# wei-zeng98/piano-a2s

Measured on AMD Instinct MI355X. Metric: training clips/sec (12 s, 5-bar), higher is better.
Workload: dtype f32

## Files before the change

piano_a2s_amd/csrc/a2s_api.hip:

```cpp
#define A2S_SWITCHES_IMPL
#include "a2s_internal.h"

thread_local char a2s_err_msg[512] = {0};
long long a2s_launch_counter = 0;

#define ST ((hipStream_t)stream)

extern "C" {

const char* a2s_last_error(void) { return a2s_err_msg; }
int a2s_version(void) { return 1; }
long long a2s_launch_count(void) { return __atomic_load_n(&a2s_launch_counter, __ATOMIC_RELAXED); }

int a2s_gemm_f32(void* stream, int M, int N, int K, float alpha, const float* A, long sAm, long sAk, const float* B, long sBk,
                 long sBn, float beta, float* C, long ldc, const float* bias, int act, int batch, long bsA, long bsB, long bsC,
                 int splitk, float* workspace, size_t workspace_bytes) {
    return a2s_gemm_impl(ST, M, N, K, alpha, A, sAm, sAk, B, sBk, sBn, beta, C, ldc, bias, act, batch, bsA, bsB, bsC, splitk,
                         workspace, workspace_bytes);
}
int a2s_gemm_f32_affine(void* stream, int M, int N, int K, float alpha, const float* A, long sAm, long sAk, const float* B, long sBk,
                        long sBn, float beta, float* C, long ldc, const float* bias, int act, int batch, long bsA, long bsB, long bsC,
                        int splitk, float* workspace, size_t workspace_bytes, const float* a_scale, const float* a_shift, int a_period,
                        const float* b_scale, const float* b_shift, int b_period) {
    return a2s_gemm_affine_impl(ST, M, N, K, alpha, A, sAm, sAk, B, sBk, sBn, beta, C, ldc, bias, act, batch, bsA, bsB, bsC, splitk,
// ... 42 lines not shown
}
int a2s_linear_fwd_eligible(int M, int N, int K, int period) { return a2s_linear_fwd_ok(M, N, K, 4, 4, period, nullptr, nullptr, nullptr) ? 1 : 0; }
int a2s_linear_dgrad_blocks(int M) { return a2s_linear_dgrad_blocks_impl(M); }
int a2s_linear_dgrad_eligible(int M, int N, int K, int period) {
    return a2s_linear_dgrad_ok(M, N, K, 4, 1, K, 4, period, nullptr, nullptr, nullptr, nullptr) ? 1 : 0;
}
int a2s_gemm_f32_bnstats(void* stream, int M, int N, int K, const float* A, long sAm, long sAk, const float* B, long sBk, long sBn, float* C, long ldc,
                         const float* y, const float* mean, const float* invstd, const float* scale, const float* shift, int period, float* partial) {
    return a2s_gemm_affine_impl(ST, M, N, K, 1.f, A, sAm, sAk, B, sBk, sBn, 0.f, C, ldc, nullptr, 0, 1, 0, 0, 0, 1, nullptr, 0,
                                nullptr, nullptr, 0, nullptr, nullptr, 0, y, mean, invstd, scale, shift, partial, period, 0, nullptr, nullptr);
}
int a2s_gemm_bnstats_blocks(int M, int period) { return a2s_cdiv(M, 128) * a2s_gemm_bnstats_slots(period); }
size_t a2s_gemm_workspace_bytes(int M, int N, int batch, int splitk) { return a2s_gemm_workspace_bytes_impl(M, N, batch, splitk); }
int a2s_gemm_pick_splitk(int M, int N, int K, int batch) { return a2s_gemm_pick_splitk_impl(M, N, K, batch); }
void a2s_gemm_debug_tile(int cfg) { a2s_gemm_debug_tile_impl(cfg); }
size_t a2s_note_step_workspace_floats(int H, int E) { return a2s_note_step_workspace_floats_impl(H, E); }
int a2s_debug_set(const char* key, int value) {
    if (!key) return A2S_ERR_ARG;
    const int id = a2s_switch_find(key);
    if (id >= 0) { a2s_switch_store(id, value); return A2S_OK; }
    if (!strcmp(key, "attn_deferred_fast")) { a2s_attn_deferred_fast = value ? 1 : 0; return A2S_OK; }
    if (!strcmp(key, "tallk_wgrad")) { a2s_tallk_wgrad_on = value ? 1 : 0; return A2S_OK; }
    if (!strcmp(key, "tallk_wgrad_max_splits")) { a2s_tallk_wgrad_max_splits = value > 0 ? value : 0; return A2S_OK; }
    if (!strcmp(key, "gemm_tile")) { a2s_gemm_debug_tile_impl(value); return A2S_OK; }
    snprintf(a2s_err_msg, sizeof(a2s_err_msg), "a2s_debug_set: unknown key %s", key);
    return A2S_ERR_ARG;
}
int a2s_env_check(void) {
    if (const char* e = a2s_switch_env_error()) A2S_FAIL(A2S_ERR_ARG, "%s: expected a decimal number >= 0", e);
    return A2S_OK;
}

int a2s_persist_abort_latch(void* device_word) { a2s_persist_latch_set(device_word); return A2S_OK; }

int a2s_debug_get(const char* key) {
    if (!key) return -1;
    const int id = a2s_switch_find(key);
    if (id == A2S_SW_attn_pair_fused_rows) return a2s_attn_pair_fused_rows();
    if (id >= 0) return a2s_sw((a2s_switch)id);
    if (!strcmp(key, "attn_pair_launches")) return (int)a2s_attn_pair_launches();
    if (!strcmp(key, "attn_pair_bwd_launches")) return (int)a2s_attn_pair_bwd_launches();
    if (!strcmp(key, "attn_deferred_fast")) return a2s_attn_deferred_fast;
    if (!strcmp(key, "tallk_wgrad")) return a2s_tallk_wgrad_on;
    if (!strcmp(key, "tallk_wgrad_max_splits")) return a2s_tallk_wgrad_max_splits;
    if (!strcmp(key, "tallk_wgrad_launches")) return (int)a2s_tallk_wgrad_launches();
    if (!strcmp(key, "attn_dk_ahead_launches")) return (int)a2s_attn_dk_ahead_launches();
    if (!strcmp(key, "attn_denc_launches")) return (int)a2s_attn_denc_launches();
    if (!strcmp(key, "dec_mid_launches")) return a2s_dec_mid_launches();
    if (!strcmp(key, "dec_cmb_launches")) return a2s_dec_cmb_launches();
    if (!strcmp(key, "dec_persist_launches")) return a2s_dec_persist_launches();
    if (!strcmp(key, "edit_distance_launches")) return (int)a2s_edit_distance_launches();
    if (!strcmp(key, "conv_rows16_c20_launches")) return (int)a2s_conv_rows16_c20_launches();
    if (!strcmp(key, "device_cus")) return a2s_device_geometry().cus;
    if (!strcmp(key, "device_xccs")) return a2s_device_geometry().xccs;
    return -1;
}

int a2s_conv3x3(void* stream, const float* x, const float* w, float* y, const float* in_scale, const float* in_shift,
                float* stat_partial, int B, int T, int F, int Cin, int Cout, int flip, float* workspace) {
    return a2s_conv3x3_impl(ST, x, w, y, in_scale, in_shift, stat_partial, B, T, F, Cin, Cout, flip, workspace, nullptr, nullptr, nullptr, nullptr, nullptr, nullptr,
                            nullptr, nullptr);
}
int a2s_conv3x3_ranged(void* stream, const float* x, const float* w, float* y, const float* in_scale, const float* in_shift, const float* in_absmax,
                       float* stat_partial, float* out_absmax, int B, int T, int F, int Cin, int Cout, float* workspace) {
    return a2s_conv3x3_impl(ST, x, w, y, in_scale, in_shift, stat_partial, B, T, F, Cin, Cout, 0, workspace, nullptr, nullptr, nullptr, nullptr, nullptr, nullptr,
                            in_absmax, out_absmax);
}
int a2s_conv3x3_dgrad_bnstats(void* stream, const float* dy, const float* w, float* g, const float* yl, const float* yl_mean, const float* yl_invstd,
                              const float* yl_scale, const float* yl_shift, float* stat_partial, int B, int T, int F, int Cin, int Cout,
                              float* workspace) {
    if (!yl) { snprintf(a2s_err_msg, sizeof(a2s_err_msg), "conv3x3_dgrad_bnstats: yl is required"); return A2S_ERR_ARG; }
    return a2s_conv3x3_impl(ST, dy, w, g, nullptr, nullptr, stat_partial, B, T, F, Cin, Cout, 1, workspace, yl, yl_mean, yl_invstd, yl_scale, yl_shift, nullptr, nullptr, nullptr);
// ... 382 lines not shown
```

piano_a2s_amd/csrc/a2s_bwd.hip:

```cpp
#include "a2s_internal.h"

__global__ __launch_bounds__(256) void log_softmax_bwd_rows(const float* __restrict__ g, const float* __restrict__ y,
                                                            long outer_stride, int inner, float* __restrict__ dx,
                                                            int R, int V, int n_outer, int time_major) {
    const int row = blockIdx.x * 4 + (threadIdx.x >> 6), lane = threadIdx.x & 63;
    if (row >= R) return;
    const int ob = row / inner, in = row % inner;
    const float* gr = g + (long)ob * outer_stride + (long)in * V;
    const float* yr = y + (long)ob * outer_stride + (long)in * V;
    float s = 0.f;
    for (int j = lane; j < V; j += 64) s += gr[j];
    s = wave_sum(s);
    const long orow = time_major ? ((long)in * n_outer + ob) : row;
    for (int j = lane; j < V; j += 64) dx[orow * V + j] = gr[j] - expf(yr[j]) * s;
}

int a2s_log_softmax_bwd_rows_impl(hipStream_t st, const float* g, const float* y, long outer_stride, int inner, float* dx,
                                  int R, int V, int n_outer, int time_major) {
    hipLaunchKernelGGL(log_softmax_bwd_rows, dim3(a2s_cdiv(R, 4)), dim3(256), 0, st, g, y, outer_stride, inner, dx, R, V, n_outer, time_major);
    A2S_CHECK_LAUNCH("log_softmax_bwd_rows");
    return A2S_OK;
}

__global__ void gru_gates_bwd(const float* __restrict__ dh_a, long lda, const float* __restrict__ dh_b, long ldb,
// ... 378 lines not shown
    hipLaunchKernelGGL(embed_scatter_add, dim3(a2s_cdiv((long)R * E, 256)), dim3(256), 0, st, table_grad, ids64, ids32, id_stride,
                       const_id, g, ldg, col0, R, E, drop, inv_keep);
    A2S_CHECK_LAUNCH("embed_scatter_add");
    return A2S_OK;
}

__global__ void ew_act_bwd(const float* __restrict__ g, const float* __restrict__ y, float* __restrict__ dx, long n, int act) {
    const long stride = (long)gridDim.x * blockDim.x;
    for (long i = (long)blockIdx.x * blockDim.x + threadIdx.x; i < n; i += stride) {
        const float yy = y[i];
        dx[i] = act == 2 ? g[i] * (1.f - yy * yy) : (yy > 0.f ? g[i] : 0.f);
    }
}
int a2s_ew_act_bwd_impl(hipStream_t st, const float* g, const float* y, float* dx, long n, int act) {
    hipLaunchKernelGGL(ew_act_bwd, dim3(min((long)2048, (n + 255) / 256)), dim3(256), 0, st, g, y, dx, n, act);
    A2S_CHECK_LAUNCH("ew_act_bwd");
    return A2S_OK;
}


static int attn_pair_bwd_sweep(hipStream_t st, const a2s_note_dec_bwd_args& au, const a2s_note_dec_bwd_args& al, int s, AttnPairStep& p);
static int attn_pair_bwd_combine(hipStream_t st, const a2s_note_dec_bwd_args& a, int s, const AttnPairStep& p);

struct NoteBwdStaff { bool mid = false; int cur = 0; int fused_rows_limit = -1; };
static int note_bwd_step_rows(const a2s_note_dec_bwd_args& a, int s) { return (a.row_list && a.n_rows_active) ? a.n_rows_active[s] : a.R; }
static bool note_bwd_step_fused(const a2s_note_dec_bwd_args& a, int s, int rows_limit) {
    const void* ptrs[] = {a.dgi_all, a.dgh_all, a.dq_all, a.dx, a.dh, a.w_ih, a.w_hh, a.attn_w};
    const int n = note_bwd_step_rows(a, s);
    if (rows_limit >= 0 && n > rows_limit) return false;
    return n > 0 && a2s_dec_step_fusable(n, a.H, a.E, 173, ptrs, 8, a.step_ws, a.step_ws_floats);
}

static int note_bwd_step(hipStream_t st, const a2s_note_dec_bwd_args& a, int s, NoteBwdStaff& c, int part, const AttnPairStep* pair) {
    const int H2 = 2 * a.H, ldx = a.E + H2, R = a.R;
    const bool fused = note_bwd_step_fused(a, s, c.fused_rows_limit);
    a2s_attn_rows rows_v = {a.clip_order, a.clip_rank, a.row_until, a.n_clips > 0 ? a.n_clips : R, a.n_active ? a.n_active[s] : 0, s};
    const a2s_attn_rows* rows = a.n_active ? &rows_v : nullptr;
    float* dh_in = a.dh + (long)c.cur * R * H2;
    float* dh_out = a.dh + (long)(c.cur ^ 1) * R * H2;
    if (fused) {
        const int nrows = note_bwd_step_rows(a, s);
        int rc = a2s_note_step_fused_bwd(st, a, s, dh_in, dh_out, rows, nrows, nrows < R ? a.row_list : nullptr);
        if (rc) return rc;
        c.cur ^= 1;
        return A2S_OK;
    }
    int gM = R, gB = 1;
    long gS = 0;
    if (a.m_active && a.n_clips > 0 && a2s_prefix_rows_ok(a.m_active[s], a.n_clips)) { gM = a.m_active[s]; gB = R / a.n_clips; gS = a.n_clips; }
    const float* dos = a.do_all + (long)s * R * 2 * H2;
    float* dgi = a.dgi_all + (long)s * R * 3 * H2;
    float* dgh = a.dgh_all + (long)s * R * 3 * H2;
    float* dxs = a.dx + (long)s * R * ldx;
    int rc = A2S_OK;
    if (part != 2) {
        rc = a2s_gru_gates_bwd_impl(st, dh_in, H2, dos, 2 * H2, a.gates + (long)s * R * 4 * H2, a.h + (long)s * R * H2, H2,
                                    dgi, 3 * H2, dgh, 3 * H2, nullptr, 0, dh_out, H2, R, H2);
        if (rc) return rc;
        if (c.mid) {
            const int nrows = note_bwd_step_rows(a, s);
            rc = a2s_note_step_mid_bwd(st, a, s, dh_out, nrows, nrows < R ? a.row_list : nullptr);
        } else {
            rc = a2s_gemm_impl(st, gM, ldx, 3 * H2, 1.f, dgi, 3 * H2, 1, a.w_ih, ldx, 1, 0.f, dxs, ldx, nullptr, 0, gB, gS * 3 * H2, 0, gS * ldx, 0, a.gemm_ws, a.gemm_ws_bytes);
        }
        if (rc) return rc;
        if (part == 1) return A2S_OK;
    }
    rc = pair ? attn_pair_bwd_combine(st, a, s, *pair)
              : a2s_attn_step_bwd_impl(st, a.keys, a.enc, a.q + (long)s * R * a.H, a.H, a.attn_v, a.attw + (long)s * R * a.T,
                                       a.x + (long)s * R * ldx + a.E, ldx, dxs + a.E, ldx, dos + H2, 2 * H2,
                                       a.dctx_all + (long)s * R * H2, H2, a.dq_all + (long)s * R * a.H, a.H,
                                       a.ds_all + (long)s * R * a.T, R, a.T, a.H, a.attn_ws, rows);
    if (rc) return rc;
    if (!c.mid) {
        rc = a2s_gemm_impl(st, gM, H2, 3 * H2, 1.f, dgh, 3 * H2, 1, a.w_hh, H2, 1, 1.f, dh_out, H2, nullptr, 0, gB, gS * 3 * H2, 0, gS * H2, 0, a.gemm_ws, a.gemm_ws_bytes);
        if (rc) return rc;
    }
    if (c.mid) {
        const int nrows = note_bwd_step_rows(a, s);
        rc = a2s_note_step_mid_bwd_query(st, a, s, dh_out, nrows, nrows < R ? a.row_list : nullptr);
    } else
    rc = a2s_gemm_impl(st, gM, H2, a.H, 1.f, a.dq_all + (long)s * R * a.H, a.H, 1, a.attn_w, 2 * H2, 1, 1.f, dh_out, H2, nullptr, 0, gB, gS * a.H, 0, gS * H2, 0, a.gemm_ws, a.gemm_ws_bytes);
    if (rc) return rc;
    c.cur ^= 1;
    return A2S_OK;
}

static int note_bwd_prepare(hipStream_t st, const a2s_note_dec_bwd_args& a, NoteBwdStaff& c) {
    const int H2 = 2 * a.H, ldx = a.E + H2, R = a.R;
    hipError_t e = hipMemsetAsync(a.dh, 0, sizeof(float) * 2 * R * H2, st);
    if (e == hipSuccess && (a.m_active || a.row_list)) e = hipMemsetAsync(a.dx, 0, sizeof(float) * (size_t)a.steps * R * ldx, st);
    if (e != hipSuccess) A2S_FAIL(A2S_ERR_HIP, "note_decoder_bwd memset: %s", hipGetErrorString(e));
    bool any_fused = false;
    for (int s = a.steps - 1; s >= 0 && !any_fused; --s) any_fused = note_bwd_step_fused(a, s, c.fused_rows_limit);
    const bool mid = a2s_note_step_mid_bwd_ok(a);
    bool any_mid = false;
    if (mid) for (int s = a.steps - 1; s >= 0 && !any_mid; --s) any_mid = !note_bwd_step_fused(a, s, c.fused_rows_limit);
    if (any_fused || any_mid) { int rc = a2s_note_step_fused_bwd_prepare(st, a); if (rc) return rc; }
    c.mid = mid;
    return A2S_OK;
}
static int note_bwd_finish(hipStream_t st, const a2s_note_dec_bwd_args& a, int cur) {
    if (cur != 0) {
        const hipError_t e = hipMemcpyAsync(a.dh, a.dh + (long)a.R * 2 * a.H, sizeof(float) * a.R * 2 * a.H, hipMemcpyDeviceToDevice, st);
        if (e != hipSuccess) A2S_FAIL(A2S_ERR_HIP, "note_decoder_bwd copy: %s", hipGetErrorString(e));
    }
    return A2S_OK;
}

int a2s_note_decoder_bwd_impl(hipStream_t st, const a2s_note_dec_bwd_args& a) {
    if (a2s_note_decoder_bwd_persist_ok(a)) return a2s_note_decoder_bwd_persist(st, a);
    NoteBwdStaff c;
    int rc = note_bwd_prepare(st, a, c);
    if (rc) return rc;
    for (int s = a.steps - 1; s >= 0; --s) {
        rc = note_bwd_step(st, a, s, c, 0, nullptr);
        if (rc) return rc;
    }
    return note_bwd_finish(st, a, c.cur);
}

// ... 967 lines not shown
```

piano_a2s_amd/csrc/a2s_internal.h:

```cpp
#pragma once
#include "a2s_common.h"
#include "../../include/a2s.h"
#include "a2s_switches.h"

static inline int a2s_attn_pair_fused_rows(void) {
    const int cap = a2s_sw(A2S_SW_dec_fused_max_rows), v = a2s_sw(A2S_SW_attn_pair_fused_rows);
    return v < cap ? v : cap;
}
static inline unsigned a2s_persist_dbg(void) {
    return (a2s_sw(A2S_SW_persist_force_agent) ? PERSIST_DBG_FORCE_AGENT : 0u) | (a2s_sw(A2S_SW_persist_inject_abort) ? PERSIST_DBG_INJECT_ABORT : 0u);
}

int a2s_absmax_impl(hipStream_t st, const float* x, long n, float* out);
size_t a2s_gemm_workspace_bytes_impl(int M, int N, int batch, int splitk);
int a2s_gemm_pick_splitk_impl(int M, int N, int K, int batch);
int a2s_gemm_bnstats_slots(int period);
void a2s_gemm_debug_tile_impl(int cfg);
int a2s_gemm_affine_impl(hipStream_t st, int M, int N, int K, float alpha, const float* A, long sAm, long sAk,
    const float* B, long sBk, long sBn, float beta, float* C, long ldc, const float* bias, int act,
    int batch, long bsA, long bsB, long bsC, int splitk, float* ws, size_t ws_bytes,
    const float* a_scale, const float* a_shift, int a_period, const float* b_scale, const float* b_shift, int b_period,
    const float* ep_y, const float* ep_mean, const float* ep_invstd, const float* ep_scale, const float* ep_shift,
    float* ep_partial, int ep_period, int two_term, const float* a_absmax, const float* b_absmax);
int a2s_gemm_impl(hipStream_t st, int M, int N, int K, float alpha, const float* A, long sAm, long sAk,
// ... 145 lines not shown
int a2s_embed_scatter_add_impl(hipStream_t st, float* table_grad, const long long* ids64, const int* ids32, long id_stride,
    int const_id, const float* g, long ldg, int col0, int R, int E, const uint8_t* drop, float inv_keep);
int a2s_ew_act_bwd_impl(hipStream_t st, const float* g, const float* y, float* dx, long n, int act);
int a2s_note_decoder_bwd_impl(hipStream_t st, const a2s_note_dec_bwd_args& a);
int a2s_note_decoder_bwd_pair_impl(hipStream_t su, hipStream_t sl, const a2s_note_dec_bwd_args& au, const a2s_note_dec_bwd_args& al, const int* pair_order,
    const int* pair_rank, const int* pair_n_active);
int a2s_gru_seq_bwd_impl(hipStream_t st, const float* dout, long do_bstride, long do_tstride, const float* out, long out_bstride,
    long out_tstride, const float* gates, const float* w_hh, const float* dhn, float* dgi_all, float* dgh_shift,
    float* dgh_first, float* dhbuf, float* dgh_tmp, int B, int T, int H, int reverse, float* ws, size_t ws_bytes,
    float* ranges_out, int* ranges_valid);
int a2s_staff_emb_bwd_impl(hipStream_t st, const float* note_emb, const float* const* w, float* const* grads_dev, float* note_emb_grad,
    const long long* ids64, const int* ids32, long id_bstride, const long long* lengths, long len_stride,
    const float* dout, long lddo, int col0, const float* hsave, int R, int maxlen, int E, int S);
long a2s_attn_pair_bwd_launches(void);

size_t a2s_note_step_fused_head_floats(void);
size_t a2s_note_step_workspace_floats_impl(int H, int E);
int a2s_dec_mid_launches(void);
int a2s_dec_cmb_launches(void);
bool a2s_dec_step_fusable(int R, int H, int E, int V, const void* const* ptrs, int nptrs, const float* ws, size_t ws_floats, bool greedy = false);
int a2s_note_step_fused_fwd(hipStream_t st, const a2s_note_dec_args& a, int si, int so, int sv, int sv_next, int t, const int* t_base, int tf, bool last,
    int nrows, const int* rowmap, const a2s_attn_deferred* defer = nullptr);
int a2s_note_step_fused_bwd_prepare(hipStream_t st, const a2s_note_dec_bwd_args& a);
int a2s_note_step_fused_bwd(hipStream_t st, const a2s_note_dec_bwd_args& a, int s, const float* dh_in, float* dh_out, const a2s_attn_rows* rows,
    int nrows, const int* rowmap);
bool a2s_note_step_mid_ok(int H, int E, const void* const* ptrs, int nptrs);
int a2s_note_step_mid_gru(hipStream_t st, const a2s_note_dec_args& a, int si, int so, int sv, int sv_next, int nrows, const int* rowmap);
bool a2s_note_step_mid_bwd_ok(const a2s_note_dec_bwd_args& a);
int a2s_note_step_mid_bwd(hipStream_t st, const a2s_note_dec_bwd_args& a, int s, float* dh_out, int nrows, const int* rowmap);
int a2s_note_step_mid_bwd_query(hipStream_t st, const a2s_note_dec_bwd_args& a, int s, float* dh_out, int nrows, const int* rowmap);

bool a2s_grammar_ref_ok(const a2s_grammar_ref& g, int R, int V);
int a2s_grammar_argmax_rows_impl(hipStream_t st, const float* x, long ldx, float* y, long ldy, const signed char* next, int n_states, int* row_state,
    int* choice_out, int R, int V);
int a2s_grammar_step_finalize_impl(hipStream_t st, const StepFinArgs& a, const a2s_grammar_ref& g);
int a2s_grammar_launches_impl(void);
bool a2s_metre_ref_ok(const a2s_metre_ref& m);
int a2s_metre_argmax_rows_impl(hipStream_t st, const float* x, long ldx, float* y, long ldy, const signed char* next, int n_states, int* row_state,
    const a2s_metre_ref* mt, int* choice_out, int R, int V);
int a2s_metre_step_finalize_impl(hipStream_t st, const StepFinArgs& a, const a2s_grammar_ref& g, const a2s_metre_ref& mt);
int a2s_metre_launches_impl(void);

int a2s_attn_align_rows_impl(hipStream_t st, const float* attw, long ldw, int R, int T, int* peak_out, float* weight_out, float* centroid_out,
    long out_stride, const int* n_done = nullptr, int n_rows_total = 0);
int a2s_align_launches_impl(void);
int a2s_note_decoder_fwd_align_impl(hipStream_t st, const a2s_note_dec_args& a, const a2s_align_args& g, int* steps_done);

int a2s_render_notes_impl(hipStream_t st, const int* programs, int rows_per_clip, int n_samples, float* wave, long wave_bstride, int B);
int a2s_render_launches_impl(void);

int a2s_transpose_targets_impl(hipStream_t st, const int* new_key, const int* interval, const int* token_map, int n_rows, int V, const int* semitones,
    const float* detune, long long* key, long long* upper, long long* lower, int bars, int U, int L, int bins_per_semitone, float* eff_bins, int* counters,
    int B);
// ... 154 lines not shown
```

piano_a2s_amd/csrc/a2s_step.hip:

```cpp
#include "a2s_internal.h"
#include <type_traits>

#define NW 8
#ifndef DEC_CH_GRU
#define DEC_CH_GRU 1
#define DEC_CH_OUT 1
#define DEC_CH_PROD 1
#define DEC_CH_QUERY 1
#endif
#ifndef DEC_NW_PROD
#define DEC_NW_PROD 8
#define DEC_NW_OUT 8
#endif

template <int NT, int CH, int NWV = NW>
__device__ __forceinline__ void mfma_rows8(const float* __restrict__ arow, const float* const (&brow)[NT], int ksteps, int wave, int lk,
                                           f32x4 (&acc)[NT]) {
    for (int u0 = wave; u0 < ksteps; u0 += NWV * CH) {
        f32x4 a[CH], b[NT][CH];
#pragma unroll
        for (int c = 0; c < CH; ++c) {
            const int u = u0 + NWV * c;
            const bool ok = u < ksteps;
            a[c] = ok ? *reinterpret_cast<const f32x4*>(arow + 16 * u + 4 * lk) : (f32x4){0.f, 0.f, 0.f, 0.f};
// ... 612 lines not shown
    float c0[2][4];
    if (!role_a) {
#pragma unroll
        for (int g = 0; g < 2; ++g)
#pragma unroll
            for (int r = 0; r < 4; ++r) c0[g][r] = a.dh[(long)dec_row(a.rowmap, min(row0 + lk * 4 + r, R - 1)) * a.H2 + min(n0 + g * 16 + li, ncols - 1)];
    }
    f32x4 acc[2] = {(f32x4){0.f, 0.f, 0.f, 0.f}, (f32x4){0.f, 0.f, 0.f, 0.f}};
    mid_product_64x32((role_a ? a.dgi : a.dgh) + (long)dec_row(a.rowmap, min(row0 + li, R - 1)) * K + 4 * lk, role_a ? a.wih_t : a.whh_t, K, n0, ncols, K, bs, acc);
#pragma unroll
    for (int g = 0; g < 2; ++g) {
        const int col = n0 + g * 16 + li;
        if (col >= ncols) continue;
#pragma unroll
        for (int r = 0; r < 4; ++r) {
            if (row0 + lk * 4 + r >= R) continue;
            const int row = dec_row(a.rowmap, row0 + lk * 4 + r);
            if (role_a) a.dx[(long)row * a.ldx + col] = acc[g][r];
            else a.dh[(long)row * a.H2 + col] = c0[g][r] + acc[g][r];
        }
    }
}

__global__ __launch_bounds__(256, MID_WAVES) void dec_bwd_query_mid(const float* __restrict__ dq, const float* __restrict__ wh_t, float* __restrict__ dh, int R, int H, int H2,
                                                         const int* __restrict__ rowmap) {
    __shared__ __attribute__((aligned(16))) float bs[2][32 * MID_LDB];
    const int lane = threadIdx.x & 63, wave = threadIdx.x >> 6;
    const int li = lane & 15, lk = lane >> 4;
    const int row0 = blockIdx.y * 64 + wave * 16, n0 = blockIdx.x * 32;
    float c0[2][4];
#pragma unroll
    for (int g = 0; g < 2; ++g)
#pragma unroll
        for (int r = 0; r < 4; ++r) c0[g][r] = dh[(long)dec_row(rowmap, min(row0 + lk * 4 + r, R - 1)) * H2 + min(n0 + g * 16 + li, H2 - 1)];
    f32x4 acc[2] = {(f32x4){0.f, 0.f, 0.f, 0.f}, (f32x4){0.f, 0.f, 0.f, 0.f}};
    mid_product_64x32(dq + (long)dec_row(rowmap, min(row0 + li, R - 1)) * H + 4 * lk, wh_t, H, n0, H2, H, bs, acc);
#pragma unroll
    for (int g = 0; g < 2; ++g) {
        const int col = n0 + g * 16 + li;
        if (col >= H2) continue;
#pragma unroll
        for (int r = 0; r < 4; ++r) {
            if (row0 + lk * 4 + r >= R) continue;
            const int row = dec_row(rowmap, row0 + lk * 4 + r);
            dh[(long)row * H2 + col] = c0[g][r] + acc[g][r];
        }
    }
}

struct DecOutqMidArgs {
    const float* o; long ldo;
    const float* out_w; const float* out_b; float* logits; long ldl; int V;
    const float* attn_w; long ld_aw; const float* attn_b; float* q_next; int H;
    const int* rowmap;
    int nva, R, H2;
};
__global__ __launch_bounds__(256, MID_WAVES) void dec_outq_mid(DecOutqMidArgs a) {
    __shared__ __attribute__((aligned(16))) float bs[2][32 * MID_LDB];
    const int lane = threadIdx.x & 63, wave = threadIdx.x >> 6;
    const int li = lane & 15, lk = lane >> 4;
    const int R = a.R, row0 = blockIdx.y * 64 + wave * 16;
    const bool role_a = (int)blockIdx.x < a.nva;
    const int n0 = (role_a ? blockIdx.x : blockIdx.x - a.nva) * 32;
    const int ncols = role_a ? a.V : a.H;
    float bias[2];
#pragma unroll
    for (int g = 0; g < 2; ++g) bias[g] = (role_a ? a.out_b : a.attn_b)[min(n0 + g * 16 + li, ncols - 1)];
    f32x4 acc[2] = {(f32x4){0.f, 0.f, 0.f, 0.f}, (f32x4){0.f, 0.f, 0.f, 0.f}};
    mid_product_64x32(a.o + (long)dec_row(a.rowmap, min(row0 + li, R - 1)) * a.ldo + 4 * lk, role_a ? a.out_w : a.attn_w, role_a ? 2L * a.H2 : a.ld_aw, n0, ncols,
                      role_a ? 2 * a.H2 : a.H2, bs, acc);
#pragma unroll
    for (int g = 0; g < 2; ++g) {
        const int col = n0 + g * 16 + li;
        if (col >= ncols) continue;
#pragma unroll
        for (int r = 0; r < 4; ++r) {
            if (row0 + lk * 4 + r >= R) continue;
            const int row = dec_row(a.rowmap, row0 + lk * 4 + r);
            if (role_a) a.logits[(long)row * a.ldl + col] = acc[g][r] + bias[g];
            else a.q_next[(long)row * a.H + col] = acc[g][r] + bias[g];
        }
    }
}

__global__ __launch_bounds__(64 * NW) void dec_bwd_query(const float* __restrict__ dq, const float* __restrict__ wh_t, float* __restrict__ dh,
                                                         int R, int H, int H2, const int* __restrict__ rowmap) {
    __shared__ f32x4 part[4 * 2 * 64];
    const int tid = threadIdx.x, lane = tid & 63, wave = tid >> 6;
    const int li = lane & 15, lk = lane >> 4;
    const int row0 = blockIdx.y * 16, n0 = blockIdx.x * 32;
    const float* brow[2];
#pragma unroll
    for (int g = 0; g < 2; ++g) brow[g] = wh_t + (long)min(n0 + g * 16 + li, H2 - 1) * H;
    float c0[2][4];
    if (wave == 0) {
#pragma unroll
        for (int g = 0; g < 2; ++g)
#pragma unroll
            for (int r = 0; r < 4; ++r) c0[g][r] = dh[(long)dec_row(rowmap, min(row0 + lk * 4 + r, R - 1)) * H2 + min(n0 + g * 16 + li, H2 - 1)];
    }
    f32x4 acc[2] = {(f32x4){0.f, 0.f, 0.f, 0.f}, (f32x4){0.f, 0.f, 0.f, 0.f}};
    mfma_rows8<2, DEC_CH_QUERY>(dq + (long)dec_row(rowmap, min(row0 + li, R - 1)) * H, brow, H / 16, wave, lk, acc);
    reduce_waves<2>(acc, part, wave, lane);
    if (wave > 0) return;
#pragma unroll
    for (int g = 0; g < 2; ++g) {
        const int col = n0 + g * 16 + li;
        if (col >= H2) continue;
#pragma unroll
        for (int r = 0; r < 4; ++r) {
            if (row0 + lk * 4 + r < R) dh[(long)dec_row(rowmap, row0 + lk * 4 + r) * H2 + col] = c0[g][r] + acc[g][r];
        }
    }
}

__global__ void transpose_ld(const float* __restrict__ in, long ld, float* __restrict__ out, int rows, int cols) {
    const long i = (long)blockIdx.x * blockDim.x + threadIdx.x;
    if (i >= (long)rows * cols) return;
    const int c = (int)(i / rows), r = (int)(i % rows);
    out[i] = in[(long)r * ld + c];
}

#define FUSED_MAX_ROWS_CAP 2048
#define FUSED_HEAD (16 + FUSED_MAX_ROWS_CAP / 16 + (long)FUSED_MAX_ROWS_CAP * 16 * NTV)
size_t a2s_note_step_fused_head_floats(void) { return (size_t)FUSED_HEAD; }
size_t a2s_note_step_workspace_floats_impl(int H, int E) {
    const long H2 = 2L * H, kx = E + H2;
    return (size_t)(FUSED_HEAD + kx * 3 * H2 + H2 * 3 * H2 + H2 * H);
}
static bool aligned16(const void* p) { return ((uintptr_t)p & 15) == 0; }
static int g_dec_mid_launches = 0;
int a2s_dec_mid_launches(void) { return g_dec_mid_launches; }
static int g_dec_cmb_launches = 0;
int a2s_dec_cmb_launches(void) { return g_dec_cmb_launches; }
static bool dec_use_mid(int nrows, int H2) { return a2s_sw(A2S_SW_dec_mid) && nrows > 160 && H2 % MID_KC == 0; }
bool a2s_dec_step_fusable(int R, int H, int E, int V, const void* const* ptrs, int nptrs, const float* ws, size_t ws_floats, bool greedy) {
// ... 42 lines not shown
    f.t_base = t_base; f.row_until = a.n_active ? a.row_until : nullptr; f.skip = greedy ? flags : nullptr;
    f.hnew = g.hout; f.attn_w = a.attn_w; f.ld_aw = 2 * H2; f.attn_b = a.attn_b;
    f.q_next = last ? nullptr : a.q + (long)sv_next * R * a.H; f.H = a.H;
    f.rowmap = rowmap;
    f.n_clips = a.n_clips > 0 ? a.n_clips : R; f.R = nrows; f.V = a.V; f.E = a.E; f.t = t; f.teacher_force = tf; f.eos_id = a.eos_id;
    f.max_t = a.steps; f.H2 = H2;
    hipLaunchKernelGGL(dec_out_step, dim3(a2s_cdiv(nrows, 16), NVW + a2s_cdiv(a.H, 32)), dim3(64 * DEC_NW_OUT), 0, st, f);
    A2S_CHECK_LAUNCH("dec_out_step");
    return A2S_OK;
}

int a2s_note_step_fused_bwd_prepare(hipStream_t st, const a2s_note_dec_bwd_args& a) {
    const int H2 = 2 * a.H, kx = a.E + H2;
    float* wih_t = a.step_ws + FUSED_HEAD;
    float* whh_t = wih_t + (long)kx * 3 * H2;
    float* wh_t = whh_t + (long)H2 * 3 * H2;
    hipLaunchKernelGGL(transpose_ld, dim3(a2s_cdiv((long)3 * H2 * kx, 256)), dim3(256), 0, st, a.w_ih, (long)kx, wih_t, 3 * H2, kx);
    hipLaunchKernelGGL(transpose_ld, dim3(a2s_cdiv((long)3 * H2 * H2, 256)), dim3(256), 0, st, a.w_hh, (long)H2, whh_t, 3 * H2, H2);
    hipLaunchKernelGGL(transpose_ld, dim3(a2s_cdiv((long)a.H * H2, 256)), dim3(256), 0, st, a.attn_w, (long)2 * H2, wh_t, a.H, H2);
    A2S_CHECK_LAUNCH("transpose_ld");
    return A2S_OK;
}

int a2s_note_step_fused_bwd(hipStream_t st, const a2s_note_dec_bwd_args& a, int s, const float* dh_in, float* dh_out, const a2s_attn_rows* rows,
                            int nrows, const int* rowmap) {
    const int H2 = 2 * a.H, ldx = a.E + H2, R = a.R;
    const float* dos = a.do_all + (long)s * R * 2 * H2;
    float* dgi = a.dgi_all + (long)s * R * 3 * H2;
    float* dgh = a.dgh_all + (long)s * R * 3 * H2;
    float* dxs = a.dx + (long)s * R * ldx;
    float* wih_t = a.step_ws + FUSED_HEAD;
    float* whh_t = wih_t + (long)ldx * 3 * H2;
    float* wh_t = whh_t + (long)H2 * 3 * H2;
    DecBwdProdArgs p;
    p.dgi = dgi; p.dgh = dgh; p.wih_t = wih_t; p.whh_t = whh_t; p.dx = dxs; p.ldx = ldx; p.dh = dh_out;
    p.rowmap = rowmap;
    p.nxa = a2s_cdiv(ldx, 32); p.kx = ldx; p.R = nrows; p.H2 = H2;
    const bool mid = dec_use_mid(nrows, H2);
    int rc = a2s_gru_gates_bwd_impl(st, dh_in, H2, dos, 2 * H2, a.gates + (long)s * R * 4 * H2, a.h + (long)s * R * H2, H2,
                                    dgi, 3 * H2, dgh, 3 * H2, nullptr, 0, dh_out, H2, R, H2);
    if (rc) return rc;
    if (mid) { hipLaunchKernelGGL(dec_bwd_mid, dim3(p.nxa + a2s_cdiv(H2, 32), a2s_cdiv(nrows, 64)), dim3(256), 0, st, p); __atomic_fetch_add(&g_dec_mid_launches, 1, __ATOMIC_RELAXED); }
    else hipLaunchKernelGGL(dec_bwd_products, dim3(p.nxa + a2s_cdiv(H2, 32), a2s_cdiv(nrows, 16)), dim3(64 * DEC_NW_PROD), 0, st, p);
    A2S_CHECK_LAUNCH("dec_bwd_products");
    rc = a2s_attn_step_bwd_impl(st, a.keys, a.enc, a.q + (long)s * R * a.H, a.H, a.attn_v, a.attw + (long)s * R * a.T,
                                a.x + (long)s * R * ldx + a.E, ldx, dxs + a.E, ldx, dos + H2, 2 * H2,
                                a.dctx_all + (long)s * R * H2, H2, a.dq_all + (long)s * R * a.H, a.H,
                                a.ds_all + (long)s * R * a.T, R, a.T, a.H, a.attn_ws, rows);
    if (rc) return rc;
    if (mid) hipLaunchKernelGGL(dec_bwd_query_mid, dim3(a2s_cdiv(H2, 32), a2s_cdiv(nrows, 64)), dim3(256), 0, st, a.dq_all + (long)s * R * a.H, wh_t, dh_out, nrows, a.H, H2, rowmap);
    else hipLaunchKernelGGL(dec_bwd_query, dim3(a2s_cdiv(H2, 32), a2s_cdiv(nrows, 16)), dim3(64 * NW), 0, st, a.dq_all + (long)s * R * a.H, wh_t, dh_out, nrows, a.H, H2,
                            rowmap);
    A2S_CHECK_LAUNCH("dec_bwd_query");
    return A2S_OK;
}


bool a2s_note_step_mid_ok(int H, int E, const void* const* ptrs, int nptrs) {
    if (!a2s_sw(A2S_SW_dec_mid) || H % MID_KC || E % 16) return false;
    for (int i = 0; i < nptrs; ++i) if (!aligned16(ptrs[i])) return false;
    return true;
}
int a2s_note_step_mid_gru(hipStream_t st, const a2s_note_dec_args& a, int si, int so, int sv, int sv_next, int nrows, const int* rowmap) {
    const int H2 = 2 * a.H, ldx = a.E + H2, R = a.R;
    if (nrows <= 0) return A2S_OK;
    DecGruArgs g;
    g.x = a.x + (long)si * R * ldx; g.ldx = ldx; g.kx = ldx;
    g.h = a.h + (long)si * R * H2;
    g.w_ih = a.w_ih; g.w_hh = a.w_hh; g.b_ih = a.b_ih; g.b_hh = a.b_hh;
    g.hout = a.h + (long)so * R * H2; g.o = a.o + (long)sv * R * 2 * H2; g.ldo = 2 * H2;
    g.save = a.gates ? a.gates + (long)sv * R * 4 * H2 : nullptr;
    g.n_done = nullptr; g.skip = nullptr;
    g.rowmap = rowmap;
    g.R = nrows; g.H2 = H2;
    hipLaunchKernelGGL(dec_gru_mid, dim3(H2 / 16, a2s_cdiv(nrows, 64)), dim3(256), 0, st, g);
// ... 6 lines not shown
    f.nva = a2s_cdiv(a.V, 32); f.R = nrows; f.H2 = H2;
    hipLaunchKernelGGL(dec_outq_mid, dim3(f.nva + (f.q_next ? a2s_cdiv(a.H, 32) : 0), a2s_cdiv(nrows, 64)), dim3(256), 0, st, f);
    A2S_CHECK_LAUNCH("dec_outq_mid");
    return A2S_OK;
}
bool a2s_note_step_mid_bwd_ok(const a2s_note_dec_bwd_args& a) {
    const void* ptrs[] = {a.dgi_all, a.dgh_all, a.dx, a.dh, a.step_ws};
    return a.step_ws && a.step_ws_floats >= a2s_note_step_workspace_floats_impl(a.H, a.E) && a2s_note_step_mid_ok(a.H, a.E, ptrs, 5);
}
int a2s_note_step_mid_bwd(hipStream_t st, const a2s_note_dec_bwd_args& a, int s, float* dh_out, int nrows, const int* rowmap) {
    const int H2 = 2 * a.H, ldx = a.E + H2, R = a.R;
    if (nrows <= 0) return A2S_OK;
    DecBwdProdArgs p;
    p.dgi = a.dgi_all + (long)s * R * 3 * H2; p.dgh = a.dgh_all + (long)s * R * 3 * H2;
    p.wih_t = a.step_ws + FUSED_HEAD; p.whh_t = p.wih_t + (long)ldx * 3 * H2;
    p.dx = a.dx + (long)s * R * ldx; p.ldx = ldx; p.dh = dh_out;
    p.rowmap = rowmap;
    p.nxa = a2s_cdiv(ldx, 32); p.kx = ldx; p.R = nrows; p.H2 = H2;
    hipLaunchKernelGGL(dec_bwd_mid, dim3(p.nxa + a2s_cdiv(H2, 32), a2s_cdiv(nrows, 64)), dim3(256), 0, st, p);
    __atomic_fetch_add(&g_dec_mid_launches, 1, __ATOMIC_RELAXED);
    A2S_CHECK_LAUNCH("dec_bwd_mid");
    return A2S_OK;
}
int a2s_note_step_mid_bwd_query(hipStream_t st, const a2s_note_dec_bwd_args& a, int s, float* dh_out, int nrows, const int* rowmap) {
    const int H2 = 2 * a.H, ldx = a.E + H2, R = a.R;
    if (nrows <= 0) return A2S_OK;
    const float* wh_t = a.step_ws + FUSED_HEAD + (long)ldx * 3 * H2 + (long)H2 * 3 * H2;
    hipLaunchKernelGGL(dec_bwd_query_mid, dim3(a2s_cdiv(H2, 32), a2s_cdiv(nrows, 64)), dim3(256), 0, st, a.dq_all + (long)s * R * a.H, wh_t, dh_out, nrows, a.H, H2, rowmap);
    A2S_CHECK_LAUNCH("dec_bwd_query_mid");
    return A2S_OK;
}
```

Measured before the change: 638.4.

## Fold next step's GRU gate backward into the decoder query-gradient kernel

Fuses the GRU gate backward of step s-1 into the epilogue of the dh query-gradient kernel of step s, so the separate gates kernel launch per decoder step is skipped. The query kernels extend their grid to cover the previous step's active rows and compute dgi/dgh/dh_next from the just-finished carry. In exchange, dgi_all/dgh_all are memset up front when row lists are used, and the query kernels grow in registers and work. It also adds a sync in the non-mid path.

```diff
diff --git a/piano_a2s_amd/csrc/a2s_api.hip b/piano_a2s_amd/csrc/a2s_api.hip
--- a/piano_a2s_amd/csrc/a2s_api.hip
+++ b/piano_a2s_amd/csrc/a2s_api.hip
@@ -88,6 +88,7 @@
     if (!strcmp(key, "attn_deferred_fast")) { a2s_attn_deferred_fast = value ? 1 : 0; return A2S_OK; }
     if (!strcmp(key, "tallk_wgrad")) { a2s_tallk_wgrad_on = value ? 1 : 0; return A2S_OK; }
     if (!strcmp(key, "tallk_wgrad_max_splits")) { a2s_tallk_wgrad_max_splits = value > 0 ? value : 0; return A2S_OK; }
+    if (!strcmp(key, "dec_bwd_fold")) { a2s_dec_bwd_fold = value ? 1 : 0; return A2S_OK; }
     if (!strcmp(key, "gemm_tile")) { a2s_gemm_debug_tile_impl(value); return A2S_OK; }
     snprintf(a2s_err_msg, sizeof(a2s_err_msg), "a2s_debug_set: unknown key %s", key);
     return A2S_ERR_ARG;
@@ -114,6 +115,8 @@
     if (!strcmp(key, "attn_denc_launches")) return (int)a2s_attn_denc_launches();
     if (!strcmp(key, "dec_mid_launches")) return a2s_dec_mid_launches();
     if (!strcmp(key, "dec_cmb_launches")) return a2s_dec_cmb_launches();
+    if (!strcmp(key, "dec_bwd_fold")) return a2s_dec_bwd_fold;
+    if (!strcmp(key, "dec_bwd_fold_launches")) return a2s_dec_bwd_fold_launches();
     if (!strcmp(key, "dec_persist_launches")) return a2s_dec_persist_launches();
     if (!strcmp(key, "edit_distance_launches")) return (int)a2s_edit_distance_launches();
     if (!strcmp(key, "conv_rows16_c20_launches")) return (int)a2s_conv_rows16_c20_launches();
diff --git a/piano_a2s_amd/csrc/a2s_bwd.hip b/piano_a2s_amd/csrc/a2s_bwd.hip
--- a/piano_a2s_amd/csrc/a2s_bwd.hip
+++ b/piano_a2s_amd/csrc/a2s_bwd.hip
@@ -424,8 +424,13 @@
 static int attn_pair_bwd_sweep(hipStream_t st, const a2s_note_dec_bwd_args& au, const a2s_note_dec_bwd_args& al, int s, AttnPairStep& p);
 static int attn_pair_bwd_combine(hipStream_t st, const a2s_note_dec_bwd_args& a, int s, const AttnPairStep& p);
 
-struct NoteBwdStaff { bool mid = false; int cur = 0; int fused_rows_limit = -1; };
+struct NoteBwdStaff { bool mid = false; int cur = 0; int fused_rows_limit = -1; bool gates_done = false; };
 static int note_bwd_step_rows(const a2s_note_dec_bwd_args& a, int s) { return (a.row_list && a.n_rows_active) ? a.n_rows_active[s] : a.R; }
+static int note_bwd_fold_rows(const a2s_note_dec_bwd_args& a, int s, int nrows) {
+    if (!a2s_dec_bwd_fold || s <= 0 || nrows <= 0) return 0;
+    const int next = note_bwd_step_rows(a, s - 1);
+    return next >= nrows ? next : 0;
+}
 static bool note_bwd_step_fused(const a2s_note_dec_bwd_args& a, int s, int rows_limit) {
     const void* ptrs[] = {a.dgi_all, a.dgh_all, a.dq_all, a.dx, a.dh, a.w_ih, a.w_hh, a.attn_w};
     const int n = note_bwd_step_rows(a, s);
@@ -441,9 +446,10 @@
     float* dh_in = a.dh + (long)c.cur * R * H2;
     float* dh_out = a.dh + (long)(c.cur ^ 1) * R * H2;
     if (fused) {
-        const int nrows = note_bwd_step_rows(a, s);
-        int rc = a2s_note_step_fused_bwd(st, a, s, dh_in, dh_out, rows, nrows, nrows < R ? a.row_list : nullptr);
+        const int nrows = note_bwd_step_rows(a, s), fold_rows = note_bwd_fold_rows(a, s, nrows);
+        int rc = a2s_note_step_fused_bwd(st, a, s, dh_in, dh_out, rows, nrows, nrows < R ? a.row_list : nullptr, c.gates_done, fold_rows);
         if (rc) return rc;
+        c.gates_done = fold_rows > 0;
         c.cur ^= 1;
         return A2S_OK;
     }
@@ -456,8 +462,10 @@
     float* dxs = a.dx + (long)s * R * ldx;
     int rc = A2S_OK;
     if (part != 2) {
-        rc = a2s_gru_gates_bwd_impl(st, dh_in, H2, dos, 2 * H2, a.gates + (long)s * R * 4 * H2, a.h + (long)s * R * H2, H2,
-                                    dgi, 3 * H2, dgh, 3 * H2, nullptr, 0, dh_out, H2, R, H2);
+        if (!c.gates_done)
+            rc = a2s_gru_gates_bwd_impl(st, dh_in, H2, dos, 2 * H2, a.gates + (long)s * R * 4 * H2, a.h + (long)s * R * H2, H2,
+                                        dgi, 3 * H2, dgh, 3 * H2, nullptr, 0, dh_out, H2, R, H2);
+        c.gates_done = false;
         if (rc) return rc;
         if (c.mid) {
             const int nrows = note_bwd_step_rows(a, s);
@@ -479,8 +487,9 @@
         if (rc) return rc;
     }
     if (c.mid) {
-        const int nrows = note_bwd_step_rows(a, s);
-        rc = a2s_note_step_mid_bwd_query(st, a, s, dh_out, nrows, nrows < R ? a.row_list : nullptr);
+        const int nrows = note_bwd_step_rows(a, s), fold_rows = note_bwd_fold_rows(a, s, nrows);
+        rc = a2s_note_step_mid_bwd_query(st, a, s, dh_in, dh_out, nrows, nrows < R ? a.row_list : nullptr, fold_rows);
+        c.gates_done = rc == A2S_OK && fold_rows > 0;
     } else
     rc = a2s_gemm_impl(st, gM, H2, a.H, 1.f, a.dq_all + (long)s * R * a.H, a.H, 1, a.attn_w, 2 * H2, 1, 1.f, dh_out, H2, nullptr, 0, gB, gS * a.H, 0, gS * H2, 0, a.gemm_ws, a.gemm_ws_bytes);
     if (rc) return rc;
@@ -499,6 +508,12 @@
     bool any_mid = false;
     if (mid) for (int s = a.steps - 1; s >= 0 && !any_mid; --s) any_mid = !note_bwd_step_fused(a, s, c.fused_rows_limit);
     if (any_fused || any_mid) { int rc = a2s_note_step_fused_bwd_prepare(st, a); if (rc) return rc; }
+    if (a2s_dec_bwd_fold && (any_fused || any_mid) && a.row_list && a.n_rows_active) {
+        const size_t nb = sizeof(float) * (size_t)a.steps * R * 3 * H2;
+        e = hipMemsetAsync(a.dgi_all, 0, nb, st);
+        if (e == hipSuccess) e = hipMemsetAsync(a.dgh_all, 0, nb, st);
+        if (e != hipSuccess) A2S_FAIL(A2S_ERR_HIP, "note_decoder_bwd memset: %s", hipGetErrorString(e));
+    }
     c.mid = mid;
     return A2S_OK;
 }
diff --git a/piano_a2s_amd/csrc/a2s_internal.h b/piano_a2s_amd/csrc/a2s_internal.h
--- a/piano_a2s_amd/csrc/a2s_internal.h
+++ b/piano_a2s_amd/csrc/a2s_internal.h
@@ -191,13 +191,15 @@
 int a2s_note_step_fused_fwd(hipStream_t st, const a2s_note_dec_args& a, int si, int so, int sv, int sv_next, int t, const int* t_base, int tf, bool last,
     int nrows, const int* rowmap, const a2s_attn_deferred* defer = nullptr);
 int a2s_note_step_fused_bwd_prepare(hipStream_t st, const a2s_note_dec_bwd_args& a);
-int a2s_note_step_fused_bwd(hipStream_t st, const a2s_note_dec_bwd_args& a, int s, const float* dh_in, float* dh_out, const a2s_attn_rows* rows,
-    int nrows, const int* rowmap);
+extern int a2s_dec_bwd_fold;
+int a2s_dec_bwd_fold_launches(void);
+int a2s_note_step_fused_bwd(hipStream_t st, const a2s_note_dec_bwd_args& a, int s, float* dh_in, float* dh_out, const a2s_attn_rows* rows,
+    int nrows, const int* rowmap, bool gates_done, int fold_rows);
 bool a2s_note_step_mid_ok(int H, int E, const void* const* ptrs, int nptrs);
 int a2s_note_step_mid_gru(hipStream_t st, const a2s_note_dec_args& a, int si, int so, int sv, int sv_next, int nrows, const int* rowmap);
 bool a2s_note_step_mid_bwd_ok(const a2s_note_dec_bwd_args& a);
 int a2s_note_step_mid_bwd(hipStream_t st, const a2s_note_dec_bwd_args& a, int s, float* dh_out, int nrows, const int* rowmap);
-int a2s_note_step_mid_bwd_query(hipStream_t st, const a2s_note_dec_bwd_args& a, int s, float* dh_out, int nrows, const int* rowmap);
+int a2s_note_step_mid_bwd_query(hipStream_t st, const a2s_note_dec_bwd_args& a, int s, float* dh_in, float* dh_out, int nrows, const int* rowmap, int fold_rows);
 
 bool a2s_grammar_ref_ok(const a2s_grammar_ref& g, int R, int V);
 int a2s_grammar_argmax_rows_impl(hipStream_t st, const float* x, long ldx, float* y, long ldy, const signed char* next, int n_states, int* row_state,
diff --git a/piano_a2s_amd/csrc/a2s_step.hip b/piano_a2s_amd/csrc/a2s_step.hip
--- a/piano_a2s_amd/csrc/a2s_step.hip
+++ b/piano_a2s_amd/csrc/a2s_step.hip
@@ -658,28 +658,64 @@
     }
 }
 
+struct DecBwdFold {
+    const float* dos;
+    const float* gates; const float* hprev;
+    float* dgi; float* dgh;
+    float* dh_next;
+    int rows;
+};
+struct DecFoldIn { float rg, zg, ng, ghn, dout, hp; };
+__device__ __forceinline__ DecFoldIn dec_fold_load(const DecBwdFold& f, int row, int col, int H2) {
+    const float* s = f.gates + (long)row * 4 * H2;
+    return {s[col], s[H2 + col], s[2 * H2 + col], s[3 * H2 + col], f.dos[(long)row * 2 * H2 + col], f.hprev[(long)row * H2 + col]};
+}
+__device__ __forceinline__ void dec_fold_gates(const DecBwdFold& f, const DecFoldIn& v, int row, int col, int H2, float carry) {
+    const GruCellGrad cg = gru_cell_bwd(carry + v.dout, v.rg, v.zg, v.ng, v.ghn, v.hp);
+    float* a = f.dgi + (long)row * 3 * H2;
+    a[col] = cg.dr; a[H2 + col] = cg.dz; a[2 * H2 + col] = cg.dn;
+    float* b = f.dgh + (long)row * 3 * H2;
+    b[col] = cg.dr; b[H2 + col] = cg.dz; b[2 * H2 + col] = cg.dnr;
+    f.dh_next[(long)row * H2 + col] = cg.dhz;
+}
+
 __global__ __launch_bounds__(256, MID_WAVES) void dec_bwd_query_mid(const float* __restrict__ dq, const float* __restrict__ wh_t, float* __restrict__ dh, int R, int H, int H2,
-                                                         const int* __restrict__ rowmap) {
+                                                         const int* __restrict__ rowmap, DecBwdFold f) {
     __shared__ __attribute__((aligned(16))) float bs[2][32 * MID_LDB];
     const int lane = threadIdx.x & 63, wave = threadIdx.x >> 6;
     const int li = lane & 15, lk = lane >> 4;
     const int row0 = blockIdx.y * 64 + wave * 16, n0 = blockIdx.x * 32;
+    const int RT = f.dos && f.rows > R ? f.rows : R;
     float c0[2][4];
 #pragma unroll
     for (int g = 0; g < 2; ++g)
 #pragma unroll
-        for (int r = 0; r < 4; ++r) c0[g][r] = dh[(long)dec_row(rowmap, min(row0 + lk * 4 + r, R - 1)) * H2 + min(n0 + g * 16 + li, H2 - 1)];
+        for (int r = 0; r < 4; ++r) c0[g][r] = dh[(long)dec_row(rowmap, min(row0 + lk * 4 + r, RT - 1)) * H2 + min(n0 + g * 16 + li, H2 - 1)];
     f32x4 acc[2] = {(f32x4){0.f, 0.f, 0.f, 0.f}, (f32x4){0.f, 0.f, 0.f, 0.f}};
-    mid_product_64x32(dq + (long)dec_row(rowmap, min(row0 + li, R - 1)) * H + 4 * lk, wh_t, H, n0, H2, H, bs, acc);
+    if ((int)blockIdx.y * 64 < R)
+        mid_product_64x32(dq + (long)dec_row(rowmap, min(row0 + li, R - 1)) * H + 4 * lk, wh_t, H, n0, H2, H, bs, acc);
+    int rows[4];
+#pragma unroll
+    for (int r = 0; r < 4; ++r) rows[r] = dec_row(rowmap, min(row0 + lk * 4 + r, RT - 1));
+    DecFoldIn fv[2][4] = {};
+    if (f.dos) {
+#pragma unroll
+        for (int g = 0; g < 2; ++g)
+#pragma unroll
+            for (int r = 0; r < 4; ++r)
+                if (n0 + g * 16 + li < H2 && row0 + lk * 4 + r < RT) fv[g][r] = dec_fold_load(f, rows[r], n0 + g * 16 + li, H2);
+    }
 #pragma unroll
     for (int g = 0; g < 2; ++g) {
         const int col = n0 + g * 16 + li;
         if (col >= H2) continue;
 #pragma unroll
         for (int r = 0; r < 4; ++r) {
-            if (row0 + lk * 4 + r >= R) continue;
-            const int row = dec_row(rowmap, row0 + lk * 4 + r);
-            dh[(long)row * H2 + col] = c0[g][r] + acc[g][r];
+            const int ri = row0 + lk * 4 + r;
+            if (ri >= RT) continue;
+            float carry = c0[g][r];
+            if (ri < R) { carry += acc[g][r]; dh[(long)rows[r] * H2 + col] = carry; }
+            if (f.dos) dec_fold_gates(f, fv[g][r], rows[r], col, H2, carry);
         }
     }
 }
@@ -720,11 +756,19 @@
 }
 
 __global__ __launch_bounds__(64 * NW) void dec_bwd_query(const float* __restrict__ dq, const float* __restrict__ wh_t, float* __restrict__ dh,
-                                                         int R, int H, int H2, const int* __restrict__ rowmap) {
+                                                         int R, int H, int H2, const int* __restrict__ rowmap, DecBwdFold f) {
     __shared__ f32x4 part[4 * 2 * 64];
+    __shared__ float carry[16 * 32];
     const int tid = threadIdx.x, lane = tid & 63, wave = tid >> 6;
     const int li = lane & 15, lk = lane >> 4;
     const int row0 = blockIdx.y * 16, n0 = blockIdx.x * 32;
+    const bool fold = f.dos != nullptr;
+    const int RT = fold && f.rows > R ? f.rows : R;
+    const int fi = row0 + (tid >> 5), fcol = n0 + (tid & 31);
+    const bool fmine = fold && fi < RT && fcol < H2;
+    const int frow = fmine ? dec_row(rowmap, fi) : 0;
+    DecFoldIn fv = {};
+    if (fmine) fv = dec_fold_load(f, frow, fcol, H2);
     const float* brow[2];
 #pragma unroll
     for (int g = 0; g < 2; ++g) brow[g] = wh_t + (long)min(n0 + g * 16 + li, H2 - 1) * H;
@@ -733,21 +777,33 @@
 #pragma unroll
         for (int g = 0; g < 2; ++g)
 #pragma unroll
-            for (int r = 0; r < 4; ++r) c0[g][r] = dh[(long)dec_row(rowmap, min(row0 + lk * 4 + r, R - 1)) * H2 + min(n0 + g * 16 + li, H2 - 1)];
+            for (int r = 0; r < 4; ++r) c0[g][r] = dh[(long)dec_row(rowmap, min(row0 + lk * 4 + r, RT - 1)) * H2 + min(n0 + g * 16 + li, H2 - 1)];
     }
     f32x4 acc[2] = {(f32x4){0.f, 0.f, 0.f, 0.f}, (f32x4){0.f, 0.f, 0.f, 0.f}};
-    mfma_rows8<2, DEC_CH_QUERY>(dq + (long)dec_row(rowmap, min(row0 + li, R - 1)) * H, brow, H / 16, wave, lk, acc);
-    reduce_waves<2>(acc, part, wave, lane);
-    if (wave > 0) return;
-#pragma unroll
-    for (int g = 0; g < 2; ++g) {
-        const int col = n0 + g * 16 + li;
-        if (col >= H2) continue;
-#pragma unroll
-        for (int r = 0; r < 4; ++r) {
-            if (row0 + lk * 4 + r < R) dh[(long)dec_row(rowmap, row0 + lk * 4 + r) * H2 + col] = c0[g][r] + acc[g][r];
-        }
-    }
+    if (row0 < R) {
+        mfma_rows8<2, DEC_CH_QUERY>(dq + (long)dec_row(rowmap, min(row0 + li, R - 1)) * H, brow, H / 16, wave, lk, acc);
+        reduce_waves<2>(acc, part, wave, lane);
+    }
+    if (wave > 0 && !fold) return;
+    if (wave == 0) {
+#pragma unroll
+        for (int g = 0; g < 2; ++g) {
+            const int col = n0 + g * 16 + li;
+#pragma unroll
+            for (int r = 0; r < 4; ++r) {
+                const int ri = row0 + lk * 4 + r;
+                float c = c0[g][r];
+                if (ri < R) {
+                    c += acc[g][r];
+                    if (col < H2) dh[(long)dec_row(rowmap, ri) * H2 + col] = c;
+                }
+                if (fold) carry[(lk * 4 + r) * 32 + g * 16 + li] = c;
+            }
+        }
+    }
+    if (!fold) return;
+    __syncthreads();
+    if (fmine) dec_fold_gates(f, fv, frow, fcol, H2, carry[(tid >> 5) * 32 + (tid & 31)]);
 }
 
 __global__ void transpose_ld(const float* __restrict__ in, long ld, float* __restrict__ out, int rows, int cols) {
@@ -836,9 +892,25 @@
     return A2S_OK;
 }
 
-int a2s_note_step_fused_bwd(hipStream_t st, const a2s_note_dec_bwd_args& a, int s, const float* dh_in, float* dh_out, const a2s_attn_rows* rows,
-                            int nrows, const int* rowmap) {
+int a2s_dec_bwd_fold = 1;
+static int g_dec_bwd_fold_launches = 0;
+int a2s_dec_bwd_fold_launches(void) { return g_dec_bwd_fold_launches; }
+static DecBwdFold dec_bwd_fold_args(const a2s_note_dec_bwd_args& a, int s, float* dh_next, int fold_rows) {
+    const long H2 = 2 * a.H, R = a.R;
+    DecBwdFold f = {};
+    if (fold_rows <= 0) return f;
+    f.dos = a.do_all + (s - 1) * R * 2 * H2;
+    f.gates = a.gates + (s - 1) * R * 4 * H2; f.hprev = a.h + (s - 1) * R * H2;
+    f.dgi = a.dgi_all + (s - 1) * R * 3 * H2; f.dgh = a.dgh_all + (s - 1) * R * 3 * H2;
+    f.dh_next = dh_next; f.rows = fold_rows;
+    __atomic_fetch_add(&g_dec_bwd_fold_launches, 1, __ATOMIC_RELAXED);
+    return f;
+}
+
+int a2s_note_step_fused_bwd(hipStream_t st, const a2s_note_dec_bwd_args& a, int s, float* dh_in, float* dh_out, const a2s_attn_rows* rows,
+                            int nrows, const int* rowmap, bool gates_done, int fold_rows) {
     const int H2 = 2 * a.H, ldx = a.E + H2, R = a.R;
+    A2S_REQUIRE(fold_rows <= 0 || (s > 0 && fold_rows >= nrows && (rowmap || fold_rows == nrows)), "note_step_fused_bwd: fold over %d rows behind a step of %d", fold_rows, nrows);
     const float* dos = a.do_all + (long)s * R * 2 * H2;
     float* dgi = a.dgi_all + (long)s * R * 3 * H2;
     float* dgh = a.dgh_all + (long)s * R * 3 * H2;
@@ -851,8 +923,8 @@
     p.rowmap = rowmap;
     p.nxa = a2s_cdiv(ldx, 32); p.kx = ldx; p.R = nrows; p.H2 = H2;
     const bool mid = dec_use_mid(nrows, H2);
-    int rc = a2s_gru_gates_bwd_impl(st, dh_in, H2, dos, 2 * H2, a.gates + (long)s * R * 4 * H2, a.h + (long)s * R * H2, H2,
-                                    dgi, 3 * H2, dgh, 3 * H2, nullptr, 0, dh_out, H2, R, H2);
+    int rc = gates_done ? A2S_OK : a2s_gru_gates_bwd_impl(st, dh_in, H2, dos, 2 * H2, a.gates + (long)s * R * 4 * H2, a.h + (long)s * R * H2, H2,
+                                                          dgi, 3 * H2, dgh, 3 * H2, nullptr, 0, dh_out, H2, R, H2);
     if (rc) return rc;
     if (mid) { hipLaunchKernelGGL(dec_bwd_mid, dim3(p.nxa + a2s_cdiv(H2, 32), a2s_cdiv(nrows, 64)), dim3(256), 0, st, p); __atomic_fetch_add(&g_dec_mid_launches, 1, __ATOMIC_RELAXED); }
     else hipLaunchKernelGGL(dec_bwd_products, dim3(p.nxa + a2s_cdiv(H2, 32), a2s_cdiv(nrows, 16)), dim3(64 * DEC_NW_PROD), 0, st, p);
@@ -862,9 +934,11 @@
                                 a.dctx_all + (long)s * R * H2, H2, a.dq_all + (long)s * R * a.H, a.H,
                                 a.ds_all + (long)s * R * a.T, R, a.T, a.H, a.attn_ws, rows);
     if (rc) return rc;
-    if (mid) hipLaunchKernelGGL(dec_bwd_query_mid, dim3(a2s_cdiv(H2, 32), a2s_cdiv(nrows, 64)), dim3(256), 0, st, a.dq_all + (long)s * R * a.H, wh_t, dh_out, nrows, a.H, H2, rowmap);
-    else hipLaunchKernelGGL(dec_bwd_query, dim3(a2s_cdiv(H2, 32), a2s_cdiv(nrows, 16)), dim3(64 * NW), 0, st, a.dq_all + (long)s * R * a.H, wh_t, dh_out, nrows, a.H, H2,
-                            rowmap);
+    const DecBwdFold f = dec_bwd_fold_args(a, s, dh_in, fold_rows);
+    const int grows = fold_rows > nrows ? fold_rows : nrows;
+    if (mid) hipLaunchKernelGGL(dec_bwd_query_mid, dim3(a2s_cdiv(H2, 32), a2s_cdiv(grows, 64)), dim3(256), 0, st, a.dq_all + (long)s * R * a.H, wh_t, dh_out, nrows, a.H, H2, rowmap, f);
+    else hipLaunchKernelGGL(dec_bwd_query, dim3(a2s_cdiv(H2, 32), a2s_cdiv(grows, 16)), dim3(64 * NW), 0, st, a.dq_all + (long)s * R * a.H, wh_t, dh_out, nrows, a.H, H2,
+                            rowmap, f);
     A2S_CHECK_LAUNCH("dec_bwd_query");
     return A2S_OK;
 }
@@ -917,11 +991,15 @@
     A2S_CHECK_LAUNCH("dec_bwd_mid");
     return A2S_OK;
 }
-int a2s_note_step_mid_bwd_query(hipStream_t st, const a2s_note_dec_bwd_args& a, int s, float* dh_out, int nrows, const int* rowmap) {
+int a2s_note_step_mid_bwd_query(hipStream_t st, const a2s_note_dec_bwd_args& a, int s, float* dh_in, float* dh_out, int nrows, const int* rowmap, int fold_rows) {
     const int H2 = 2 * a.H, ldx = a.E + H2, R = a.R;
+    A2S_REQUIRE(fold_rows <= 0 || (s > 0 && nrows > 0 && fold_rows >= nrows && (rowmap || fold_rows == nrows)), "note_step_mid_bwd_query: fold over %d rows behind a step of %d",
+                fold_rows, nrows);
     if (nrows <= 0) return A2S_OK;
     const float* wh_t = a.step_ws + FUSED_HEAD + (long)ldx * 3 * H2 + (long)H2 * 3 * H2;
-    hipLaunchKernelGGL(dec_bwd_query_mid, dim3(a2s_cdiv(H2, 32), a2s_cdiv(nrows, 64)), dim3(256), 0, st, a.dq_all + (long)s * R * a.H, wh_t, dh_out, nrows, a.H, H2, rowmap);
+    const DecBwdFold f = dec_bwd_fold_args(a, s, dh_in, fold_rows);
+    const int grows = fold_rows > nrows ? fold_rows : nrows;
+    hipLaunchKernelGGL(dec_bwd_query_mid, dim3(a2s_cdiv(H2, 32), a2s_cdiv(grows, 64)), dim3(256), 0, st, a.dq_all + (long)s * R * a.H, wh_t, dh_out, nrows, a.H, H2, rowmap, f);
     A2S_CHECK_LAUNCH("dec_bwd_query_mid");
     return A2S_OK;
 }
```

Result: no change. 642.1, median of 6 (+0.6%).
